# zju3dv/neuralbody

Measured on AMD Instinct MI355X. Metric: ray_samples_per_sec, higher is better.
Workload: dtype f16+f6/f4

## Files before the change

### neuralbody_amd/csrc/nb_march_common.h

```cpp
#pragma once
#include "nb_common.h"

typedef float f32x4 __attribute__((ext_vector_type(4)));
typedef float f32x16 __attribute__((ext_vector_type(16)));

namespace nbm {

constexpr int N_PE = 45;

constexpr int TAP_F = 0, TAP_H1 = 352, TAP_H2 = 608, TAP_H3 = 864, TAP_G = 1120, TAP_V = 1376, TAP_PE = 1504, TAP_WIDTH = 1600;

__device__ __forceinline__ float relu1(float x) {
    float r;
    asm("v_max_f32 %0, 0, %1" : "=v"(r) : "v"(x));
    return r;
}

__host__ __device__ constexpr int tile_row(int r, int hi) { return (r & 3) + 8 * (r >> 2) + 4 * hi; }

__host__ __device__ constexpr int lvl_c(int l) { return l == 0 ? 32 : (l == 1 ? 64 : 128); }
__host__ __device__ constexpr int lvl_chan_base(int l) { return l == 0 ? 0 : (l == 1 ? 32 : (l == 2 ? 96 : 224)); }
__host__ __device__ constexpr int lvl_reg_base(int l) { return lvl_chan_base(l) / 2; }

__host__ __device__ inline int col_feat(int q, int hi) {
// ... 106 lines not shown
    const int *ray_order;
    long long n_slots;
    float *rgb_map, *disp_map, *acc_map, *weights, *depth_map, *raw;
    long long n_rays;
    int n_samples;
    int white_bkgd;
    const float *wpts, *viewdir;
    float *raw_out, *dbg;
    long long n_pts;
    int n_wave_groups;
    float *ill;
    int ill_cap;
};

#define NB_INV_2PI 0.15915494309189533576888376337251436
__device__ __forceinline__ float sin_rev(double u) {
    const double f = u - rint(u);
    return __builtin_amdgcn_sinf((float)f);
}
__device__ __forceinline__ void pe_view(float (&pe)[N_PE], float vx, float vy, float vz, int hi) {
    const float v[3] = {vx, vy, vz};
    const double q = hi ? 0.25 : 0.0;
#pragma unroll
    for (int a = 0; a < 3; ++a) {
        const double t = (double)v[a] * NB_INV_2PI;
#pragma unroll
        for (int k = 0; k < 4; ++k) pe[3 * k + a] = sin_rev(t * (double)(1 << k) + q);
    }
}
__device__ __forceinline__ void pe_xyz(float (&pe)[N_PE], float px, float py, float pz, float vx, float vy,
                                       float vz, int hi) {
    const float p[3] = {px, py, pz};
    const float v[3] = {vx, vy, vz};
    const double q = hi ? 0.25 : 0.0;
#pragma unroll
    for (int a = 0; a < 3; ++a) {
        const double t = (double)p[a] * NB_INV_2PI;
#pragma unroll
        for (int k = 0; k < 10; ++k) pe[12 + 3 * k + a] = sin_rev(t * (double)(1 << k) + q);
    }
#pragma unroll
    for (int a = 0; a < 3; ++a) pe[42 + a] = hi ? p[a] : v[a];
}

__device__ __forceinline__ void dump_pe(const float (&pe)[N_PE], float *dst, int hi) {
#pragma unroll
    for (int c = 0; c < N_PE; ++c) dst[col_pe(c, hi) - 256] = pe[c];
}

struct GridCoord {
    float gw, gh, gd;
};

__device__ __forceinline__ GridCoord grid_coords(const SceneDev &sc, float px, float py, float pz) {
    const Pose ps = load_pose(sc.pose);
    const float qx = px - ps.Th[0], qy = py - ps.Th[1], qz = pz - ps.Th[2];
    const float cx = fmaf(qz, ps.R[6], fmaf(qy, ps.R[3], qx * ps.R[0]));
    const float cy = fmaf(qz, ps.R[7], fmaf(qy, ps.R[4], qx * ps.R[1]));
    const float cz = fmaf(qz, ps.R[8], fmaf(qy, ps.R[5], qx * ps.R[2]));
    GridCoord g;
    g.gd = __fsub_rn(__fmul_rn(__fdiv_rn(__fdiv_rn(cz - ps.bmin[2], sc.vs[0]), sc.osh[0]), 2.f), 1.f);
    g.gh = __fsub_rn(__fmul_rn(__fdiv_rn(__fdiv_rn(cy - ps.bmin[1], sc.vs[1]), sc.osh[1]), 2.f), 1.f);
    g.gw = __fsub_rn(__fmul_rn(__fdiv_rn(__fdiv_rn(cx - ps.bmin[0], sc.vs[2]), sc.osh[2]), 2.f), 1.f);
    return g;
}

template <int L>
__device__ __forceinline__ void gather_level(const SceneDev &sc, const GridCoord &g, int hi,
                                             float (&out)[lvl_c(L) / 2]) {
    constexpr int C = lvl_c(L), HALF = C / 2;
    const int D = sc.dhw[L][0], H = sc.dhw[L][1], W = sc.dhw[L][2];
    float ix = __fmul_rn(__fdiv_rn(__fadd_rn(g.gw, 1.f), 2.f), (float)(W - 1));
    float iy = __fmul_rn(__fdiv_rn(__fadd_rn(g.gh, 1.f), 2.f), (float)(H - 1));
    float iz = __fmul_rn(__fdiv_rn(__fadd_rn(g.gd, 1.f), 2.f), (float)(D - 1));
    ix = fminf(fmaxf(ix, -2.f), (float)W + 1.f);
    iy = fminf(fmaxf(iy, -2.f), (float)H + 1.f);
    iz = fminf(fmaxf(iz, -2.f), (float)D + 1.f);
    const float fx = floorf(ix), fy = floorf(iy), fz = floorf(iz);
    const int x0 = (int)fx, y0 = (int)fy, z0 = (int)fz;
    const float wx[2] = {(fx + 1.f) - ix, ix - fx};
    const float wy[2] = {(fy + 1.f) - iy, iy - fy};
    const float wz[2] = {(fz + 1.f) - iz, iz - fz};
    const float *vb = sc.vol[L] + hi * HALF;
    const f32x4 *cp[8];
    float cw[8];
#pragma unroll
    for (int corner = 0; corner < 8; ++corner) {
        const int dx = corner & 1, dy = (corner >> 1) & 1, dz = corner >> 2;
        const int xx = x0 + dx, yy = y0 + dy, zz = z0 + dz;
        const bool inb = (unsigned)xx < (unsigned)W && (unsigned)yy < (unsigned)H && (unsigned)zz < (unsigned)D;
        cw[corner] = inb ? (wx[dx] * wy[dy]) * wz[dz] : 0.f;
        const int xc = min(max(xx, 0), W - 1), yc = min(max(yy, 0), H - 1), zc = min(max(zz, 0), D - 1);
        cp[corner] = reinterpret_cast<const f32x4 *>(vb + ((size_t)(zc * H + yc) * W + xc) * C);
    }
#pragma unroll
    for (int grp = 0; grp < HALF / 16; ++grp) {
        f32x4 v[8][4];
#pragma unroll
        for (int corner = 0; corner < 8; ++corner)
#pragma unroll
            for (int q = 0; q < 4; ++q) v[corner][q] = cp[corner][grp * 4 + q];
#pragma unroll
        for (int q = 0; q < 4; ++q) {
            f32x4 a = {0.f, 0.f, 0.f, 0.f};
#pragma unroll
            for (int corner = 0; corner < 8; ++corner) {
                a.x = fmaf(cw[corner], v[corner][q].x, a.x);
                a.y = fmaf(cw[corner], v[corner][q].y, a.y);
                a.z = fmaf(cw[corner], v[corner][q].z, a.z);
                a.w = fmaf(cw[corner], v[corner][q].w, a.w);
            }
            out[grp * 16 + q * 4 + 0] = a.x;
            out[grp * 16 + q * 4 + 1] = a.y;
            out[grp * 16 + q * 4 + 2] = a.z;
            out[grp * 16 + q * 4 + 3] = a.w;
        }
// ... 318 lines not shown
```

### neuralbody_amd/csrc/nb_march_fold.hip

```cpp
#include "nb_f6_ops.h"
#include "nb_march_hooks.h"

using namespace nbm;

namespace {

#ifndef NB_FP4_TERMS
#define NB_FP4_TERMS 3
#endif
constexpr bool FP4_K[2] = {(NB_FP4_TERMS & 1) != 0, (NB_FP4_TERMS & 2) != 0};
constexpr bool ANY_FP4 = FP4_K[0] || FP4_K[1];
constexpr int TERM_ORDER[2] = {(FP4_K[0] && !FP4_K[1]) ? 1 : 0, (FP4_K[0] && !FP4_K[1]) ? 0 : 1};
__host__ __device__ constexpr int term_pieces(int k) { return FP4_K[k] ? 1 : 2; }
__host__ __device__ constexpr int block_pieces(int mt) { return (4 * mt + mt * term_pieces(0) + mt * term_pieces(1) + 1) & ~1; }
__host__ __device__ constexpr int cross_piece(int mt, int slot, int m) {
    return 4 * mt + (slot == 0 ? 0 : mt * term_pieces(TERM_ORDER[0])) + m * term_pieces(TERM_ORDER[slot]);
}
constexpr int S_R = 8;
__host__ __device__ constexpr int phase_pieces(int nb, int mt) { return nb * block_pieces(mt); }
constexpr int N_PH = 4;
constexpr int PH_NB[N_PH] = {4, 4, 4, 2};
constexpr int PH_MT[N_PH] = {2, 2, 1, 1};
__host__ __device__ constexpr int phase_p0(int ph) {
    int p = 0;
    for (int i = 0; i < ph; ++i) p += phase_pieces(PH_NB[i], PH_MT[i]);
    return p;
}
__host__ __device__ constexpr int phase_s0(int ph) {
    int n = 0;
    for (int i = 0; i < ph; ++i) n += PH_NB[i];
    return n;
}
constexpr int P_L1 = phase_p0(0), P_L2 = phase_p0(1), P_VG = phase_p0(2), P_VP = phase_p0(3), P_TOTAL = phase_p0(4);
constexpr int N_SCALE = phase_s0(4);
constexpr int WAVE_STREAM = P_TOTAL * 1024 + ((N_SCALE * 256 + 1023) & ~1023);
static_assert(P_TOTAL == (NB_FP4_TERMS == 3 ? 132 : (NB_FP4_TERMS == 0 ? 176 : 160)), "pieces per wave per depth step");
static_assert(S_R % 2 == 0 && P_L1 % 2 == 0 && P_L2 % 2 == 0 && P_VG % 2 == 0 && P_VP % 2 == 0, "six-bit fragments on even pieces");
__host__ __device__ constexpr int phase_of_p0(int p0) { return p0 == P_L1 ? 0 : (p0 == P_L2 ? 1 : (p0 == P_VG ? 2 : 3)); }

constexpr int F_OFF_B0 = 8 * 44 * 256;
constexpr int F_OFF_B1 = F_OFF_B0 + 256 + 8 * 32 * 256;
constexpr int F_OFF_B2 = F_OFF_B1 + 256 + 8 * 32 * 256;
constexpr int F_OFF_AW = F_OFF_B2 + 256;
constexpr int F_OFF_AB = F_OFF_AW + 256;
constexpr int F_OFF_L4 = F_OFF_AB + 4;
constexpr int F_OFF_LV = F_OFF_L4 + 8 * 32 * 256;
constexpr int F_OFF_BV = F_OFF_LV + 4 * 44 * 256;
constexpr int F_OFF_RW = F_OFF_BV + 128;
constexpr int F_OFF_RB = F_OFF_RW + 384;

constexpr int CH_BYTES = 2048;
constexpr int ACT16_BYTES = 16 * CH_BYTES;
constexpr int F6_BYTES = 2048;
constexpr int ACT6_OFF = ACT16_BYTES;
constexpr int ACT6_BYTES = 4 * 2 * 2 * F6_BYTES;
constexpr int ACT_BYTES = ACT6_OFF + ACT6_BYTES;
constexpr int WT_CHUNK = 4096;
constexpr int U_CHUNK = 4096;
constexpr int K_CAP = 128;
constexpr int KM_CAP = 1024;
constexpr int SCR_A = ACT_BYTES;
constexpr int SCR_C = SCR_A + 1024;
// ... 256 lines not shown

typedef short s4v __attribute__((ext_vector_type(4)));
typedef __attribute__((address_space(3))) s4v *lds_s4p;

__device__ __forceinline__ float unnorm_s(float gcoord, float fm1, float fp1) {
    const float i = __fmul_rn(__fdiv_rn(__fadd_rn(gcoord, 1.f), 2.f), fm1);
    return fminf(fmaxf(i, -2.f), fp1);
}
__device__ __forceinline__ int mad24(int a, int b, int c) {
    int r;
    asm("v_mad_i32_i24 %0, %1, %2, %3" : "=v"(r) : "v"(a), "v"(b), "v"(c));
    return r;
}
template <int N>
__device__ __forceinline__ int row_ror(int v) {
    return __builtin_amdgcn_update_dpp(v, v, 0x120 | N, 0xf, 0xf, false);
}
__device__ __forceinline__ int red_min16i(int v) {
    v = min(v, row_ror<8>(v));
    v = min(v, row_ror<4>(v));
    v = min(v, row_ror<2>(v));
    v = min(v, row_ror<1>(v));
    return v;
}
__device__ __forceinline__ int red_max16i(int v) {
    v = max(v, row_ror<8>(v));
    v = max(v, row_ror<4>(v));
    v = max(v, row_ror<2>(v));
    v = max(v, row_ror<1>(v));
    return v;
}

struct Lvl {
    int D, H, W;
    float fmx, fmy, fmz, fpx, fpy, fpz;
    const int *grid;
    int rbase;
};
__device__ __forceinline__ Lvl load_lvl(const char *actz, int part) {
    const i32x4 *p = reinterpret_cast<const i32x4 *>(actz + LC_OFF + part * 48);
    const i32x4 a = p[0], b = p[1], c = p[2];
    Lvl l;
    l.D = a.x; l.H = a.y; l.W = a.z;
    l.fmx = __int_as_float(a.w); l.fmy = __int_as_float(b.x); l.fmz = __int_as_float(b.y);
    l.fpx = __int_as_float(b.z); l.fpy = __int_as_float(b.w); l.fpz = __int_as_float(c.x);
    l.grid = reinterpret_cast<const int *>(((unsigned long long)(unsigned)c.z << 32) | (unsigned long long)(unsigned)c.y);
    l.rbase = c.w;
    return l;
}
struct LvlIdx {
    float ix, iy, iz;
    int x0, y0, z0;
};
__device__ __forceinline__ LvlIdx level_index(const Lvl &lv, const GridCoord &g) {
    LvlIdx q;
    q.ix = unnorm_s(g.gw, lv.fmx, lv.fpx);
    q.iy = unnorm_s(g.gh, lv.fmy, lv.fpy);
    q.iz = unnorm_s(g.gd, lv.fmz, lv.fpz);
    q.x0 = (int)floorf(q.ix);
    q.y0 = (int)floorf(q.iy);
    q.z0 = (int)floorf(q.iz);
    return q;
}

constexpr int BOX_BIG = 1 << 24;
__device__ __forceinline__ void prep_boxes(char *actz, const Lvl &lv, const GridCoord &g, bool take, int wslot, bool write, int os, int part) {
    const LvlIdx q = level_index(lv, g);
    int xlo = take ? min(max(q.x0, 0), lv.W - 1) : BOX_BIG, xhi = take ? min(max(q.x0 + 1, 0), lv.W - 1) : -1;
    int ylo = take ? min(max(q.y0, 0), lv.H - 1) : BOX_BIG, yhi = take ? min(max(q.y0 + 1, 0), lv.H - 1) : -1;
    int zlo = take ? min(max(q.z0, 0), lv.D - 1) : BOX_BIG, zhi = take ? min(max(q.z0 + 1, 0), lv.D - 1) : -1;
    xlo = red_min16i(xlo); ylo = red_min16i(ylo); zlo = red_min16i(zlo);
    xhi = red_max16i(xhi); yhi = red_max16i(yhi); zhi = red_max16i(zhi);
    const int any = __builtin_amdgcn_ballot_w64(take) != 0ull;
    if (write && os == 0) {
        i32x4 *d = reinterpret_cast<i32x4 *>(actz + WBOX_OFF + (wslot * 4 + part) * 32);
        d[0] = i32x4{xlo, ylo, zlo, xhi};
        d[1] = i32x4{yhi, zhi, any, 0};
    }
}

struct Prep {
    int xlo, ylo, zlo, nx, nxy, n, k0;
    int K;
    int tier;
    int any;
};
__device__ __forceinline__ int box_count(int xlo, int ylo, int zlo, int xhi, int yhi, int zhi) {
    return (xhi < xlo || yhi < ylo || zhi < zlo) ? 0 : (xhi - xlo + 1) * (yhi - ylo + 1) * (zhi - zlo + 1);
}
template <int NW>
__device__ __forceinline__ Prep prep_wg(const char *actz, int part) {
    int xlo = BOX_BIG, ylo = BOX_BIG, zlo = BOX_BIG, xhi = -1, yhi = -1, zhi = -1;
    int n16[NW], any = 0;
#pragma unroll
    for (int w = 0; w < NW; ++w) {
        const i32x4 *s = reinterpret_cast<const i32x4 *>(actz + WBOX_OFF + (w * 4 + part) * 32);
        const i32x4 a = s[0], b = s[1];
        any |= b.z;
        n16[w] = box_count(a.x, a.y, a.z, a.w, b.x, b.y);
        xlo = min(xlo, a.x); ylo = min(ylo, a.y); zlo = min(zlo, a.z);
        xhi = max(xhi, a.w); yhi = max(yhi, b.x); zhi = max(zhi, b.y);
    }
    Prep p;
    p.xlo = xlo; p.ylo = ylo; p.zlo = zlo;
    p.nx = xhi - xlo + 1;
    p.nxy = p.nx * (yhi - ylo + 1);
    p.n = box_count(xlo, ylo, zlo, xhi, yhi, zhi);
    const int n0 = __builtin_amdgcn_readlane(p.n, 0), n1 = __builtin_amdgcn_readlane(p.n, 16), n2 = __builtin_amdgcn_readlane(p.n, 32),
              n3 = __builtin_amdgcn_readlane(p.n, 48);
    p.K = n0 + n1 + n2 + n3;
    p.k0 = part == 0 ? 0 : (part == 1 ? n0 : (part == 2 ? n0 + n1 : n0 + n1 + n2));
    p.tier = 0;
    p.any = any;
    if constexpr (NW > 1) {
        if (p.K > K_CAP && p.K <= KM_CAP) {
            p.tier = 3;
        } else if (p.K > K_CAP) {
            int worst = 0;
#pragma unroll
            for (int w = 0; w < NW; ++w)
                worst = max(worst, __builtin_amdgcn_readlane(n16[w], 0) + __builtin_amdgcn_readlane(n16[w], 16) +
                                       __builtin_amdgcn_readlane(n16[w], 32) + __builtin_amdgcn_readlane(n16[w], 48));
            p.tier = worst <= K_CAP ? 1 : 2;
        }
    }
    return p;
}

struct TblLoad {
    int rid[2], idx[2];
};
__device__ __forceinline__ TblLoad tbl_issue(const Prep &p, const Lvl &lv, int wave, int os) {
    TblLoad t;
    const float rcp_xy = __builtin_amdgcn_rcpf((float)max(p.nxy, 1)), rcp_x = __builtin_amdgcn_rcpf((float)max(p.nx, 1));
#pragma unroll
    for (int q = 0; q < 2; ++q) {
        const int j = 64 * q + 16 * wave + os;
        t.rid[q] = -1;
        t.idx[q] = -1;
        if (j < p.n) {
            const int vz = (int)(((float)j + 0.5f) * rcp_xy);
            const int r = mad24(vz, -p.nxy, j);
            const int vy = (int)(((float)r + 0.5f) * rcp_x);
            const int vx = mad24(vy, -p.nx, r);
            const int lin = mad24(mad24(p.zlo + vz, lv.H, p.ylo + vy), lv.W, p.xlo + vx);
            t.rid[q] = lv.grid[lin];
            t.idx[q] = p.k0 + j;
        }
    }
    return t;
}
__device__ __forceinline__ void tbl_store(char *actz, const TblLoad &t, const Lvl &lv, unsigned zero_off, int K, int tid) {
    unsigned *tbl = reinterpret_cast<unsigned *>(actz + TBL_OFF);
#pragma unroll
    for (int q = 0; q < 2; ++q)
        if (t.idx[q] >= 0) tbl[t.idx[q]] = t.rid[q] < 0 ? zero_off : (unsigned)(lv.rbase + t.rid[q]) << 10;
    if (tid < 16 && K + tid < ((K + 15) & ~15)) tbl[K + tid] = zero_off;
}
__device__ __forceinline__ void tbl_pass(char *actz, unsigned zero_off, int k_lo, int K, int tid) {
    if (tid >= K_CAP) return;
    unsigned *tbl = reinterpret_cast<unsigned *>(actz + TBL_OFF);
    const int k = k_lo + tid;
    unsigned e = zero_off;
    if (k < K) {
        const int k1 = *reinterpret_cast<const int *>(actz + LVL_OFF + 1 * 32 + 20), k2 = *reinterpret_cast<const int *>(actz + LVL_OFF + 2 * 32 + 20),
                  k3 = *reinterpret_cast<const int *>(actz + LVL_OFF + 3 * 32 + 20);
        const int L = (k >= k1) + (k >= k2) + (k >= k3);
        const i32x4 *lp = reinterpret_cast<const i32x4 *>(actz + LVL_OFF + L * 32);
        const i32x4 b0 = lp[0], b1 = lp[1];
        const Lvl lv = load_lvl(actz, L);
        const int j = k - b1.y;
        const float rcp_xy = __builtin_amdgcn_rcpf((float)max(b1.x, 1)), rcp_x = __builtin_amdgcn_rcpf((float)max(b0.w, 1));
        const int vz = (int)(((float)j + 0.5f) * rcp_xy);
        const int r = mad24(vz, -b1.x, j);
        const int vy = (int)(((float)r + 0.5f) * rcp_x);
        const int vx = mad24(vy, -b0.w, r);
        const int lin = mad24(mad24(b0.z + vz, lv.H, b0.y + vy), lv.W, b0.x + vx);
        const int rid = lv.grid[lin];
        if (rid >= 0) e = (unsigned)(lv.rbase + rid) << 10;
    }
    tbl[tid] = e;
}
__device__ __forceinline__ void lvl_store(char *actz, const Prep &p, int tid, int os, int part) {
    if (tid < 64 && os == 0) {
        i32x4 *d = reinterpret_cast<i32x4 *>(actz + LVL_OFF + part * 32);
        d[0] = i32x4{p.xlo, p.ylo, p.zlo, p.nx};
        d[1] = i32x4{p.nxy, p.k0, p.n, 0};
    }
    if (tid == 0) *reinterpret_cast<int *>(actz + HDR_OFF) = p.K;
}

struct UCfg {
    int nch, R;
    unsigned ring;
    int ring_off;
};
__device__ __forceinline__ UCfg ucfg_k(int K, unsigned lds_base, int wave);
__device__ __forceinline__ UCfg ucfg(const char *actz, unsigned lds_base, int wave) {
    return ucfg_k(__builtin_amdgcn_readfirstlane(*reinterpret_cast<const int *>(actz + HDR_OFF)), lds_base, wave);
}
__device__ __forceinline__ UCfg ucfg_k(int K, unsigned lds_base, int wave) {
    UCfg u;
// ... 185 lines not shown
        *reinterpret_cast<f32x4 *>(irec + 4) = f32x4{z_step, __fmul_rn(1e10f, recf[11]), sigma_raw, 0.f};
    } else {
        const int ch = part - 1;
        irec[8 + ch] = part == 1 ? c0.y : (part == 2 ? c0.z : c0.w);
        irec[12 + ch] = head_sum(actz, SCR_C + (ch * 64 + sample) * 16, pk[P_RB + ch]);
    }
}

__device__ __forceinline__ void composite_step(char *actz, const float *pk, int sample, int part, float z_step, float z_after, bool last,
                                               const MarchArgs &a, long long ray, int sidx, int S, bool valid, WeightStore4 &wstore, bool ins) {
    float *recf = reinterpret_cast<float *>(actz + RAY_OFF) + sample * RAY_FLOATS;
    const f32x4 c0 = *reinterpret_cast<const f32x4 *>(recf + 12);
    const float sigma_raw = ins ? head_sum(actz, SCR_A + sample * 16, pk[P_AB]) : 0.f;
    const float d = last ? 1e10f : __fsub_rn(z_after, z_step);
    const float dist = __fmul_rn(d, recf[11]);
    const float sig = fmaxf(sigma_raw, 0.f);
    const float alpha = 1.f - expf(-sig * dist);
    const float w = alpha * c0.x;
    if (part == 0) {
        const float depth = recf[16], accw = recf[17];
        recf[12] = c0.x * (__fadd_rn(__fsub_rn(1.f, alpha), 1e-10f));
        recf[16] = fmaf(w, z_step, depth);
        recf[17] = accw + w;
    } else {
        const int ch = part - 1;
        const float o = ins ? head_sum(actz, SCR_C + (ch * 64 + sample) * 16, pk[P_RB + ch]) : 0.f;
        const float col = part == 1 ? c0.y : (part == 2 ? c0.z : c0.w);
        recf[12 + part] = fmaf(w, 1.f / (1.f + expf(-o)), col);
    }
    wstore.push(a, ray, sidx, S, part, valid, w);
    if (NB_HOOK_RAW_IS_OUTPUT && a.raw && valid && part == 0) {
        float o3[3];
#pragma unroll
        for (int ch = 0; ch < 3; ++ch) o3[ch] = ins ? head_sum(actz, SCR_C + (ch * 64 + sample) * 16, pk[P_RB + ch]) : 0.f;
        *reinterpret_cast<f32x4 *>(a.raw + (ray * S + sidx) * 4) = f32x4{o3[0], o3[1], o3[2], sigma_raw};
    }
}

__host__ __device__ inline int pe_slot_col(int a, int slot) {
    if (a >= 3 || slot >= 30) return -1;
    if (slot == 0) return 256 + 27 + a;
    if (slot <= 20) {
        const int k = (slot - 1) >> 1, is_cos = (slot - 1) & 1;
        return 256 + 27 + 3 + 6 * k + 3 * is_cos + a;
    }
    if (slot == 21) return 256 + a;
    const int k = (slot - 22) >> 1, is_cos = (slot - 22) & 1;
    return 256 + 3 + 6 * k + 3 * is_cos + a;
}

template <int MODE, bool CULL>
__global__ __launch_bounds__(256, 2) void nb_march_fold_kernel(MarchArgs a, const char *stream) {
    constexpr bool POINTS = MODE != 0, DENSITY_ONLY = MODE == 2;
    static_assert(!(CULL && POINTS), "sample culling is a property of the ray march");
    saturate_fp16_conversions();
    __shared__ __attribute__((aligned(16))) char lds[LDS_BYTES];
    char *act = lds;
    const int tid = threadIdx.x;
    const int lane = threadIdx.x & 63, wave = __builtin_amdgcn_readfirstlane(threadIdx.x >> 6);
    const int grp = xcd_remap(blockIdx.x, a.n_wave_groups);
    long long ray = (long long)grp * 64 + 16 * wave + (lane & 15);
    const long long n_units = POINTS ? a.n_pts : a.n_rays;
    bool valid = ray < n_units;
    if (!valid) ray = n_units - 1;
    if (!POINTS && a.ray_order) {
        if (a.ray_order[(long long)grp * 64] == NB_SLOT_DEAD) return;
        const int v = a.ray_order[(long long)grp * 64 + 16 * wave + (lane & 15)];
        valid = v >= 0;
        ray = valid ? v : -(long long)v - 1;
    }
    const int S = POINTS ? 1 : a.n_samples;
    {
        float ox, oy, oz, dx, dy, dz, near, far, dn, vx, vy, vz;
        if constexpr (POINTS) {
            ox = a.wpts[ray * 3 + 0], oy = a.wpts[ray * 3 + 1], oz = a.wpts[ray * 3 + 2];
            dx = DENSITY_ONLY ? 0.f : a.viewdir[ray * 3 + 0], dy = DENSITY_ONLY ? 0.f : a.viewdir[ray * 3 + 1];
            dz = DENSITY_ONLY ? 1.f : a.viewdir[ray * 3 + 2];
            near = far = 0.f;
            dn = 1.f;
            vx = dx, vy = dy, vz = dz;
        } else {
            ox = a.ray_o[ray * 3 + 0], oy = a.ray_o[ray * 3 + 1], oz = a.ray_o[ray * 3 + 2];
            dx = a.ray_d[ray * 3 + 0], dy = a.ray_d[ray * 3 + 1], dz = a.ray_d[ray * 3 + 2];
            near = a.near[ray], far = a.far[ray];
            dn = sqrtf(__fadd_rn(__fadd_rn(__fmul_rn(dx, dx), __fmul_rn(dy, dy)), __fmul_rn(dz, dz)));
            vx = dx / dn, vy = dy / dn, vz = dz / dn;
        }
        if ((lane >> 4) == 0) {
            f32x4 *rec = reinterpret_cast<f32x4 *>(lds + RAY_OFF) + (16 * wave + (lane & 15)) * (RAY_FLOATS / 4);
            rec[0] = f32x4{ox, oy, oz, near};
            rec[1] = f32x4{dx, dy, dz, far};
            rec[2] = f32x4{vx, vy, vz, dn};
            rec[3] = f32x4{1.f, 0.f, 0.f, 0.f};
            rec[4] = f32x4{0.f, 0.f, 0.f, 0.f};
        }
    }
    const float *tr = (!POINTS && a.t_rand) ? a.t_rand + ray * S : nullptr;
    auto tval = [&](int s) -> float { return ((cfloat_ptr)a.t_vals)[s]; };
    auto z_at = [&](int s, float near, float far) -> float {
        if constexpr (POINTS) return 0.f;
        const float zc = z_lin(near, far, tval(s));
        if (!tr) return zc;
        const float lower = s == 0 ? zc : 0.5f * __fadd_rn(zc, z_lin(near, far, tval(s - 1)));
        const float upper = s == S - 1 ? zc : 0.5f * __fadd_rn(z_lin(near, far, tval(s + 1)), zc);
        return __fadd_rn(lower, __fmul_rn(__fsub_rn(upper, lower), tr[s]));
    };

    {
        float *prm = reinterpret_cast<float *>(lds + PRM_OFF);
        for (int i = tid; i < P_SIZE; i += 256) {
            float v;
            if (i < P_B1) v = a.pk[F_OFF_B0 + i - P_B0];
            else if (i < P_B2) v = a.pk[F_OFF_B1 + i - P_B1];
            else if (i < P_AW) v = a.pk[F_OFF_B2 + i - P_B2];
            else if (i < P_RW) v = a.pk[F_OFF_AW + i - P_AW];
            else if (i < P_AB) v = a.pk[F_OFF_RW + i - P_RW];
            else if (i < P_RB) v = a.pk[F_OFF_AB + i - P_AB];
            else if (i < P_LB) v = a.pk[F_OFF_RB + i - P_RB];
            else v = DENSITY_ONLY ? 0.f : a.lb[256 + i - P_LB];
            prm[i] = v;
        }
        if (tid < 4) {
            int *lc = reinterpret_cast<int *>(lds + LC_OFF + tid * 48);
            const unsigned long long gp = (unsigned long long)a.fold.grid[tid];
            lc[0] = a.sc.dhw[tid][0]; lc[1] = a.sc.dhw[tid][1]; lc[2] = a.sc.dhw[tid][2];
            lc[3] = __float_as_int(a.sc.fm1[tid][2]); lc[4] = __float_as_int(a.sc.fm1[tid][1]); lc[5] = __float_as_int(a.sc.fm1[tid][0]);
            lc[6] = __float_as_int(a.sc.fp1[tid][2]); lc[7] = __float_as_int(a.sc.fp1[tid][1]); lc[8] = __float_as_int(a.sc.fp1[tid][0]);
            lc[9] = (int)(unsigned)(gp & 0xffffffffull); lc[10] = (int)(unsigned)(gp >> 32);
            lc[11] = a.fold.row_base[tid];
        }
        __syncthreads();
    }
    const __amdgpu_buffer_rsrc_t wrsrc =
        __builtin_amdgcn_make_buffer_rsrc(const_cast<char *>(stream) + (size_t)wave * WAVE_STREAM, 0, WAVE_STREAM, 0x00020000);
    WRing ring;
    WeightStore4 wstore;
    typedef void __attribute__((address_space(3))) *lptr_t;
    const unsigned lds_base = (unsigned)(unsigned long long)(lptr_t)(lds);

    float z_cur;
    GridCoord g;
    bool ins = true;
    int tier, active;
    auto prep_sequential = [&](int sn, float &z_out, int lane_c) {
        const int os = lane_c & 15, part = lane_c >> 4, sample = 16 * wave + os;
        const f32x4 *rec = reinterpret_cast<const f32x4 *>(lds + RAY_OFF) + sample * (RAY_FLOATS / 4);
        const f32x4 ro = rec[0], rd = rec[1];
        z_out = z_at(sn, ro.w, rd.w);
        const float px = __fadd_rn(ro.x, __fmul_rn(rd.x, z_out)), py = __fadd_rn(ro.y, __fmul_rn(rd.y, z_out)),
                    pz = __fadd_rn(ro.z, __fmul_rn(rd.z, z_out));
        g = grid_coords(a.sc, px, py, pz);
        if constexpr (CULL) ins = cull_inside(a.cull, a.sc, px, py, pz);
        const Lvl lv = load_lvl(lds, part);
        prep_boxes(lds, lv, g, ins, wave, true, os, part);
        __syncthreads();
        const Prep pr = prep_wg<4>(lds, part);
        tier = __builtin_amdgcn_readfirstlane(pr.tier);
        active = __builtin_amdgcn_readfirstlane(pr.any);
        if (tier == 0) {
// ... 63 lines not shown
                    lvl_store(actz, pr, tid, os, part);
                    __syncthreads();
                    const UCfg u = ucfg(actz, lds_base, wave);
                    dma_initial(a, actz, lane_i, wave, u);
                    wt_build(actz, lv, g, take, wave, os, part, u.nch);
                    __syncthreads();
                    fold_mfma(a, actz, lane_i, wave, u, acc);
                    __syncthreads();
                }
            }
            FOLD_DUMP(0, 2)
            FOLD_STAMP(2);
            ring_prime<P_L1>(wl, ring);
            publish_s(actz, lane_i, wave, acc);
            FOLD_STAMP(3);
            init_bias<2>(pk + P_B1, 2 * wave, hi, acc);
            Conv6 pec;
            {
                const f32x4 ro = rec[0], rd = rec[1], rv = rec[2];
                const float xa = part == 0 ? __fadd_rn(ro.x, __fmul_rn(rd.x, z_cur))
                                           : (part == 1 ? __fadd_rn(ro.y, __fmul_rn(rd.y, z_cur)) : __fadd_rn(ro.z, __fmul_rn(rd.z, z_cur)));
                const float va = part == 0 ? rv.x : (part == 1 ? rv.y : rv.z);
                Rev2 tx, tv;
                float e[32];
                auto pe_fill = [&](auto tc) {
                    constexpr int t = decltype(tc)::value;
                    if constexpr (t == 0) {
                        tx = rev2(xa);
                        tv = rev2(va);
                        e[0] = xa;
                        e[21] = va;
                        e[30] = 0.f;
                        e[31] = 0.f;
                    } else if constexpr (t <= 10) {
                        sincos_rev2<t - 1>(tx, e[2 * t - 1], e[2 * t]);
                    } else if constexpr (t <= 14) {
                        sincos_rev2<t - 11>(tv, e[2 * t], e[2 * t + 1]);
                    } else if constexpr (t >= 16) {
                        constexpr int i = t - 16;
                        conv6_pair<2 * i>(pec, e[4 * i], e[4 * i + 1]);
                        conv6_pair<2 * i + 1>(pec, e[4 * i + 2], e[4 * i + 3]);
                    }
                };
                if constexpr (DENSITY_ONLY) layer_s<P_L1, 2, 4, true>(wl, actz, lane_i, ring, acc);
                else layer_s<P_L1, 2, 4, true>(wl, actz, lane_i, ring, acc, pe_fill);
            }
            HalfBlock peh;
            if constexpr (!DENSITY_ONLY) peh = conv6_finish(pec);
            FOLD_DUMP(1, 2)
            FOLD_STAMP(4);
            publish_s(actz, lane_i, wave, acc);
            FOLD_STAMP(5);
            init_bias<2>(pk + P_B2, 2 * wave, hi, acc);
            layer_s<P_L2, 2, 4, true>(wl, actz, lane_i, ring, acc);
            FOLD_DUMP(2, 2)
            FOLD_STAMP(6);
            if (more) {
                const f32x4 ro = rec[0], rd = rec[1];
                z_next = z_at(s + 1, ro.w, rd.w);
                const float px = __fadd_rn(ro.x, __fmul_rn(rd.x, z_next)), py = __fadd_rn(ro.y, __fmul_rn(rd.y, z_next)),
                            pz = __fadd_rn(ro.z, __fmul_rn(rd.z, z_next));
                g = grid_coords(a.sc, px, py, pz);
                if constexpr (CULL) ins = cull_inside(a.cull, a.sc, px, py, pz);
                const Lvl lv = load_lvl(actz, part);
                prep_boxes(actz, lv, g, ins, wave, true, os, part);
            }
            FOLD_STAMP(7);
            if constexpr (DENSITY_ONLY) {
#pragma unroll
                for (int m = 0; m < 2; ++m)
#pragma unroll
                    for (int n = 0; n < 2; ++n)
#pragma unroll
                        for (int r = 0; r < 16; ++r) acc[m][n][r] = relu1(acc[m][n][r]);
            } else {
                publish_s(actz, lane_i, wave, acc);
            }
            FOLD_STAMP(8);
            {
#pragma unroll
                for (int n = 0; n < 2; ++n) {
                    float s4[4] = {0.f, 0.f, 0.f, 0.f};
#pragma unroll
                    for (int m = 0; m < 2; ++m) {
                        const f32x4 *aw = reinterpret_cast<const f32x4 *>(pk + P_AW + hi * 128 + 16 * (2 * wave + m));
#pragma unroll
                        for (int q4 = 0; q4 < 4; ++q4) {
                            const f32x4 w4 = aw[q4];
                            s4[0] = fmaf(w4.x, acc[m][n][4 * q4 + 0], s4[0]);
                            s4[1] = fmaf(w4.y, acc[m][n][4 * q4 + 1], s4[1]);
                            s4[2] = fmaf(w4.z, acc[m][n][4 * q4 + 2], s4[2]);
                            s4[3] = fmaf(w4.w, acc[m][n][4 * q4 + 3], s4[3]);
                        }
                    }
                    float sa = add_halves((s4[0] + s4[1]) + (s4[2] + s4[3]));
                    if (hi == 0) reinterpret_cast<float *>(actz + SCR_A)[(n * 32 + (lane_i & 31)) * 4 + wave] = sa;
                }
            }
            if constexpr (!DENSITY_ONLY) {
                TblLoad tl;
                int k_next = 0;
                if (more) {
                    const Lvl lv = load_lvl(actz, part);
                    const Prep pr = prep_wg<4>(actz, part);
                    tier_next = __builtin_amdgcn_readfirstlane(pr.tier);
                    active_next = __builtin_amdgcn_readfirstlane(pr.any);
                    k_next = __builtin_amdgcn_readfirstlane(pr.K);
                    tl.rid[0] = tl.rid[1] = tl.idx[0] = tl.idx[1] = -1;
                    if (tier_next == 0) tl = tbl_issue(pr, lv, wave, os);
                    lvl_store(actz, pr, tid, os, part);
                }
                FOLD_STAMP(9);
                init_bias<1>(pk + P_LB, wave, hi, acc);
                layer_s<P_VG, 1, 4, false>(wl, actz, lane_i, ring, acc);
                FOLD_STAMP(10);
                if (more && tier_next == 0) {
                    const Lvl lv = load_lvl(actz, part);
                    tbl_store(actz, tl, lv, a.fold.zero_off, k_next, tid);
                }
                __syncthreads();
                ring_prime<P_VP>(wl, ring);
                store_halfblock(actz, part >> 1, part & 1, sn, ss, peh);
                __syncthreads();
                FOLD_STAMP(11);
                layer_s<P_VP, 1, 2, false>(wl, actz, lane_i, ring, acc);
                FOLD_STAMP(12);
                FOLD_DUMP(3, 1)
                {
#pragma unroll
                    for (int n = 0; n < 2; ++n) {
                        float rl[16];
#pragma unroll
                        for (int r = 0; r < 16; ++r) rl[r] = relu1(acc[0][n][r]);
#pragma unroll
                        for (int ch = 0; ch < 3; ++ch) {
                            const f32x4 *rw = reinterpret_cast<const f32x4 *>(pk + P_RW + (ch * 2 + hi) * 64 + 16 * wave);
                            float c4[4] = {0.f, 0.f, 0.f, 0.f};
#pragma unroll
                            for (int q4 = 0; q4 < 4; ++q4) {
                                const f32x4 w4 = rw[q4];
                                c4[0] = fmaf(w4.x, rl[4 * q4 + 0], c4[0]);
                                c4[1] = fmaf(w4.y, rl[4 * q4 + 1], c4[1]);
                                c4[2] = fmaf(w4.z, rl[4 * q4 + 2], c4[2]);
                                c4[3] = fmaf(w4.w, rl[4 * q4 + 3], c4[3]);
                            }
                            float sc = add_halves((c4[0] + c4[1]) + (c4[2] + c4[3]));
                            if (hi == 0) reinterpret_cast<float *>(actz + SCR_C)[(ch * 64 + n * 32 + (lane_i & 31)) * 4 + wave] = sc;
                        }
                    }
                }
            }
        } else if (more) {
            prep_sequential(s + 1, z_next, lane_i);
            tier_next = tier;
            active_next = active;
        }
        FOLD_STAMP(13);
        __syncthreads();
        FOLD_STAMP(14);
        if (more) {
            tier = tier_next;
            active = active_next;
            fetch_and_weights(lane_i);
        }
        FOLD_STAMP(15);
        {
            if constexpr (POINTS) {
// ... 289 lines not shown
```

Measured before the change: 1.399 billion.

## Interleave next-sample coordinate and box prep into MFMA layer loops

Splits the next-sample position, grid-coordinate and per-axis box computation into small steps and passes them as fill callbacks into the FC2 layer loop. It also splits the workgroup box merge, k-list prep and table gather issue into steps run inside the VG layer loop. The aim is to hide scalar and latency-bound work under matrix instructions instead of running it serially between layers. The cost is higher register pressure and a more complex schedule, and the change depends on layer_s accepting a fill functor, which is not shown.

```diff
diff --git a/neuralbody_amd/csrc/nb_march_common.h b/neuralbody_amd/csrc/nb_march_common.h
--- a/neuralbody_amd/csrc/nb_march_common.h
+++ b/neuralbody_amd/csrc/nb_march_common.h
@@ -182,16 +182,26 @@
     float gw, gh, gd;
 };
 
-__device__ __forceinline__ GridCoord grid_coords(const SceneDev &sc, float px, float py, float pz) {
+struct CanonRel {
+    float d, h, w;
+};
+__device__ __forceinline__ CanonRel grid_canon_rel(const SceneDev &sc, float px, float py, float pz) {
     const Pose ps = load_pose(sc.pose);
     const float qx = px - ps.Th[0], qy = py - ps.Th[1], qz = pz - ps.Th[2];
     const float cx = fmaf(qz, ps.R[6], fmaf(qy, ps.R[3], qx * ps.R[0]));
     const float cy = fmaf(qz, ps.R[7], fmaf(qy, ps.R[4], qx * ps.R[1]));
     const float cz = fmaf(qz, ps.R[8], fmaf(qy, ps.R[5], qx * ps.R[2]));
+    return CanonRel{cz - ps.bmin[2], cy - ps.bmin[1], cx - ps.bmin[0]};
+}
+__device__ __forceinline__ float grid_axis_voxels(float rel, float vs) { return __fdiv_rn(rel, vs); }
+__device__ __forceinline__ float grid_axis_norm(float voxels, float osh) { return __fsub_rn(__fmul_rn(__fdiv_rn(voxels, osh), 2.f), 1.f); }
+
+__device__ __forceinline__ GridCoord grid_coords(const SceneDev &sc, float px, float py, float pz) {
+    const CanonRel c = grid_canon_rel(sc, px, py, pz);
     GridCoord g;
-    g.gd = __fsub_rn(__fmul_rn(__fdiv_rn(__fdiv_rn(cz - ps.bmin[2], sc.vs[0]), sc.osh[0]), 2.f), 1.f);
-    g.gh = __fsub_rn(__fmul_rn(__fdiv_rn(__fdiv_rn(cy - ps.bmin[1], sc.vs[1]), sc.osh[1]), 2.f), 1.f);
-    g.gw = __fsub_rn(__fmul_rn(__fdiv_rn(__fdiv_rn(cx - ps.bmin[0], sc.vs[2]), sc.osh[2]), 2.f), 1.f);
+    g.gd = grid_axis_norm(grid_axis_voxels(c.d, sc.vs[0]), sc.osh[0]);
+    g.gh = grid_axis_norm(grid_axis_voxels(c.h, sc.vs[1]), sc.osh[1]);
+    g.gw = grid_axis_norm(grid_axis_voxels(c.w, sc.vs[2]), sc.osh[2]);
     return g;
 }
 
diff --git a/neuralbody_amd/csrc/nb_march_fold.hip b/neuralbody_amd/csrc/nb_march_fold.hip
--- a/neuralbody_amd/csrc/nb_march_fold.hip
+++ b/neuralbody_amd/csrc/nb_march_fold.hip
@@ -8,6 +8,10 @@
 #ifndef NB_FP4_TERMS
 #define NB_FP4_TERMS 3
 #endif
+#ifndef NB_MARCH_FILLS
+#define NB_MARCH_FILLS 3
+#endif
+constexpr bool FILL_FC2 = (NB_MARCH_FILLS & 1) != 0, FILL_VG = (NB_MARCH_FILLS & 2) != 0;
 constexpr bool FP4_K[2] = {(NB_FP4_TERMS & 1) != 0, (NB_FP4_TERMS & 2) != 0};
 constexpr bool ANY_FP4 = FP4_K[0] || FP4_K[1];
 constexpr int TERM_ORDER[2] = {(FP4_K[0] && !FP4_K[1]) ? 1 : 0, (FP4_K[0] && !FP4_K[1]) ? 0 : 1};
@@ -370,31 +374,63 @@
     float ix, iy, iz;
     int x0, y0, z0;
 };
+__device__ __forceinline__ void level_axis(float gcoord, float fm1, float fp1, float &i, int &i0) {
+    i = unnorm_s(gcoord, fm1, fp1);
+    i0 = (int)floorf(i);
+}
 __device__ __forceinline__ LvlIdx level_index(const Lvl &lv, const GridCoord &g) {
     LvlIdx q;
-    q.ix = unnorm_s(g.gw, lv.fmx, lv.fpx);
-    q.iy = unnorm_s(g.gh, lv.fmy, lv.fpy);
-    q.iz = unnorm_s(g.gd, lv.fmz, lv.fpz);
-    q.x0 = (int)floorf(q.ix);
-    q.y0 = (int)floorf(q.iy);
-    q.z0 = (int)floorf(q.iz);
+    level_axis(g.gw, lv.fmx, lv.fpx, q.ix, q.x0);
+    level_axis(g.gh, lv.fmy, lv.fpy, q.iy, q.y0);
+    level_axis(g.gd, lv.fmz, lv.fpz, q.iz, q.z0);
     return q;
 }
 
 constexpr int BOX_BIG = 1 << 24;
+struct Box {
+    int xlo, ylo, zlo, xhi, yhi, zhi;
+};
+__device__ __forceinline__ void box_clamp(int i0, int size, bool take, int &lo, int &hi) {
+    lo = take ? min(max(i0, 0), size - 1) : BOX_BIG;
+    hi = take ? min(max(i0 + 1, 0), size - 1) : -1;
+}
+__device__ __forceinline__ int wave_takes_any(bool take) { return __builtin_amdgcn_ballot_w64(take) != 0ull; }
 __device__ __forceinline__ void prep_boxes(char *actz, const Lvl &lv, const GridCoord &g, bool take, int wslot, bool write, int os, int part) {
     const LvlIdx q = level_index(lv, g);
-    int xlo = take ? min(max(q.x0, 0), lv.W - 1) : BOX_BIG, xhi = take ? min(max(q.x0 + 1, 0), lv.W - 1) : -1;
-    int ylo = take ? min(max(q.y0, 0), lv.H - 1) : BOX_BIG, yhi = take ? min(max(q.y0 + 1, 0), lv.H - 1) : -1;
-    int zlo = take ? min(max(q.z0, 0), lv.D - 1) : BOX_BIG, zhi = take ? min(max(q.z0 + 1, 0), lv.D - 1) : -1;
-    xlo = red_min16i(xlo); ylo = red_min16i(ylo); zlo = red_min16i(zlo);
-    xhi = red_max16i(xhi); yhi = red_max16i(yhi); zhi = red_max16i(zhi);
-    const int any = __builtin_amdgcn_ballot_w64(take) != 0ull;
+    Box b;
+    box_clamp(q.x0, lv.W, take, b.xlo, b.xhi);
+    box_clamp(q.y0, lv.H, take, b.ylo, b.yhi);
+    box_clamp(q.z0, lv.D, take, b.zlo, b.zhi);
+    b.xlo = red_min16i(b.xlo); b.ylo = red_min16i(b.ylo); b.zlo = red_min16i(b.zlo);
+    b.xhi = red_max16i(b.xhi); b.yhi = red_max16i(b.yhi); b.zhi = red_max16i(b.zhi);
+    const int any = wave_takes_any(take);
     if (write && os == 0) {
         i32x4 *d = reinterpret_cast<i32x4 *>(actz + WBOX_OFF + (wslot * 4 + part) * 32);
-        d[0] = i32x4{xlo, ylo, zlo, xhi};
-        d[1] = i32x4{yhi, zhi, any, 0};
-    }
+        d[0] = i32x4{b.xlo, b.ylo, b.zlo, b.xhi};
+        d[1] = i32x4{b.yhi, b.zhi, any, 0};
+    }
+}
+template <int AX>
+__device__ __forceinline__ void box_axis_own(const char *actz, int part, float gcoord, bool take, int &lo, int &hi) {
+    const int *lc = reinterpret_cast<const int *>(actz + LC_OFF + part * 48);
+    float i;
+    int i0;
+    level_axis(gcoord, __int_as_float(lc[3 + AX]), __int_as_float(lc[6 + AX]), i, i0);
+    box_clamp(i0, lc[2 - AX], take, lo, hi);
+}
+template <int AX>
+__device__ __forceinline__ void box_axis_store(char *actz, int lo, int hi, int wslot, bool write, int os, int part) {
+    lo = red_min16i(lo);
+    hi = red_max16i(hi);
+    if (write && os == 0) {
+        int *d = reinterpret_cast<int *>(actz + WBOX_OFF + (wslot * 4 + part) * 32);
+        d[AX] = lo;
+        d[3 + AX] = hi;
+    }
+}
+__device__ __forceinline__ void box_any_store(char *actz, bool take, int wslot, bool write, int os, int part) {
+    const int any = wave_takes_any(take);
+    if (write && os == 0) reinterpret_cast<int *>(actz + WBOX_OFF + (wslot * 4 + part) * 32)[6] = any;
 }
 
 struct Prep {
@@ -407,18 +443,32 @@
     return (xhi < xlo || yhi < ylo || zhi < zlo) ? 0 : (xhi - xlo + 1) * (yhi - ylo + 1) * (zhi - zlo + 1);
 }
 template <int NW>
+struct WgBox {
+    Box b = {BOX_BIG, BOX_BIG, BOX_BIG, -1, -1, -1};
+    int n16[NW], any = 0;
+};
+template <int NW>
+__device__ __forceinline__ void wg_box_merge(const char *actz, int part, int w, WgBox<NW> &m) {
+    const i32x4 *s = reinterpret_cast<const i32x4 *>(actz + WBOX_OFF + (w * 4 + part) * 32);
+    const i32x4 a = s[0], b = s[1];
+    m.any |= b.z;
+    m.n16[w] = box_count(a.x, a.y, a.z, a.w, b.x, b.y);
+    m.b.xlo = min(m.b.xlo, a.x); m.b.ylo = min(m.b.ylo, a.y); m.b.zlo = min(m.b.zlo, a.z);
+    m.b.xhi = max(m.b.xhi, a.w); m.b.yhi = max(m.b.yhi, b.x); m.b.zhi = max(m.b.zhi, b.y);
+}
+template <int NW>
+__device__ __forceinline__ Prep prep_wg_finish(const WgBox<NW> &m, int part);
+template <int NW>
 __device__ __forceinline__ Prep prep_wg(const char *actz, int part) {
-    int xlo = BOX_BIG, ylo = BOX_BIG, zlo = BOX_BIG, xhi = -1, yhi = -1, zhi = -1;
-    int n16[NW], any = 0;
-#pragma unroll
-    for (int w = 0; w < NW; ++w) {
-        const i32x4 *s = reinterpret_cast<const i32x4 *>(actz + WBOX_OFF + (w * 4 + part) * 32);
-        const i32x4 a = s[0], b = s[1];
-        any |= b.z;
-        n16[w] = box_count(a.x, a.y, a.z, a.w, b.x, b.y);
-        xlo = min(xlo, a.x); ylo = min(ylo, a.y); zlo = min(zlo, a.z);
-        xhi = max(xhi, a.w); yhi = max(yhi, b.x); zhi = max(zhi, b.y);
-    }
+    WgBox<NW> m;
+#pragma unroll
+    for (int w = 0; w < NW; ++w) wg_box_merge(actz, part, w, m);
+    return prep_wg_finish(m, part);
+}
+template <int NW>
+__device__ __forceinline__ Prep prep_wg_finish(const WgBox<NW> &m, int part) {
+    const int xlo = m.b.xlo, ylo = m.b.ylo, zlo = m.b.zlo, xhi = m.b.xhi, yhi = m.b.yhi, zhi = m.b.zhi, any = m.any;
+    const int(&n16)[NW] = m.n16;
     Prep p;
     p.xlo = xlo; p.ylo = ylo; p.zlo = zlo;
     p.nx = xhi - xlo + 1;
@@ -448,24 +498,25 @@
 struct TblLoad {
     int rid[2], idx[2];
 };
+__device__ __forceinline__ void tbl_issue_one(TblLoad &t, int q, const Prep &p, const Lvl &lv, int wave, int os) {
+    const float rcp_xy = __builtin_amdgcn_rcpf((float)max(p.nxy, 1)), rcp_x = __builtin_amdgcn_rcpf((float)max(p.nx, 1));
+    const int j = 64 * q + 16 * wave + os;
+    t.rid[q] = -1;
+    t.idx[q] = -1;
+    if (j < p.n) {
+        const int vz = (int)(((float)j + 0.5f) * rcp_xy);
+        const int r = mad24(vz, -p.nxy, j);
+        const int vy = (int)(((float)r + 0.5f) * rcp_x);
+        const int vx = mad24(vy, -p.nx, r);
+        const int lin = mad24(mad24(p.zlo + vz, lv.H, p.ylo + vy), lv.W, p.xlo + vx);
+        t.rid[q] = lv.grid[lin];
+        t.idx[q] = p.k0 + j;
+    }
+}
 __device__ __forceinline__ TblLoad tbl_issue(const Prep &p, const Lvl &lv, int wave, int os) {
     TblLoad t;
-    const float rcp_xy = __builtin_amdgcn_rcpf((float)max(p.nxy, 1)), rcp_x = __builtin_amdgcn_rcpf((float)max(p.nx, 1));
-#pragma unroll
-    for (int q = 0; q < 2; ++q) {
-        const int j = 64 * q + 16 * wave + os;
-        t.rid[q] = -1;
-        t.idx[q] = -1;
-        if (j < p.n) {
-            const int vz = (int)(((float)j + 0.5f) * rcp_xy);
-            const int r = mad24(vz, -p.nxy, j);
-            const int vy = (int)(((float)r + 0.5f) * rcp_x);
-            const int vx = mad24(vy, -p.nx, r);
-            const int lin = mad24(mad24(p.zlo + vz, lv.H, p.ylo + vy), lv.W, p.xlo + vx);
-            t.rid[q] = lv.grid[lin];
-            t.idx[q] = p.k0 + j;
-        }
-    }
+    tbl_issue_one(t, 0, p, lv, wave, os);
+    tbl_issue_one(t, 1, p, lv, wave, os);
     return t;
 }
 __device__ __forceinline__ void tbl_store(char *actz, const TblLoad &t, const Lvl &lv, unsigned zero_off, int K, int tid) {
@@ -757,6 +808,7 @@
 template <int MODE, bool CULL>
 __global__ __launch_bounds__(256, 2) void nb_march_fold_kernel(MarchArgs a, const char *stream) {
     constexpr bool POINTS = MODE != 0, DENSITY_ONLY = MODE == 2;
+    constexpr bool FILL_KLIST = FILL_VG && !CULL;
     static_assert(!(CULL && POINTS), "sample culling is a property of the ray march");
     saturate_fp16_conversions();
     __shared__ __attribute__((aligned(16))) char lds[LDS_BYTES];
@@ -802,14 +854,15 @@
     }
     const float *tr = (!POINTS && a.t_rand) ? a.t_rand + ray * S : nullptr;
     auto tval = [&](int s) -> float { return ((cfloat_ptr)a.t_vals)[s]; };
-    auto z_at = [&](int s, float near, float far) -> float {
+    auto z_at_t = [&](int s, float near, float far, float trs) -> float {
         if constexpr (POINTS) return 0.f;
         const float zc = z_lin(near, far, tval(s));
         if (!tr) return zc;
         const float lower = s == 0 ? zc : 0.5f * __fadd_rn(zc, z_lin(near, far, tval(s - 1)));
         const float upper = s == S - 1 ? zc : 0.5f * __fadd_rn(z_lin(near, far, tval(s + 1)), zc);
-        return __fadd_rn(lower, __fmul_rn(__fsub_rn(upper, lower), tr[s]));
+        return __fadd_rn(lower, __fmul_rn(__fsub_rn(upper, lower), trs));
     };
+    auto z_at = [&](int s, float near, float far) -> float { return z_at_t(s, near, far, (!POINTS && tr) ? tr[s] : 0.f); };
 
     {
         float *prm = reinterpret_cast<float *>(lds + PRM_OFF);
@@ -979,10 +1032,60 @@
             publish_s(actz, lane_i, wave, acc);
             FOLD_STAMP(5);
             init_bias<2>(pk + P_B2, 2 * wave, hi, acc);
-            layer_s<P_L2, 2, 4, true>(wl, actz, lane_i, ring, acc);
+            if constexpr (POINTS || !FILL_FC2) {
+                layer_s<P_L2, 2, 4, true>(wl, actz, lane_i, ring, acc);
+            } else {
+                const int s1 = more ? s + 1 : s;
+                f32x4 ro, rd;
+                float trn = 0.f, px, py, pz, vox;
+                CanonRel cr;
+                int lo, hi2;
+                auto next_fill = [&](auto tc) {
+                    constexpr int t = decltype(tc)::value;
+                    if constexpr (t == 0) {
+                        ro = rec[0], rd = rec[1];
+                        if (tr) trn = tr[s1];
+                    } else if constexpr (t == 1) {
+                        z_next = z_at_t(s1, ro.w, rd.w, trn);
+                        px = __fadd_rn(ro.x, __fmul_rn(rd.x, z_next)), py = __fadd_rn(ro.y, __fmul_rn(rd.y, z_next)),
+                        pz = __fadd_rn(ro.z, __fmul_rn(rd.z, z_next));
+                    } else if constexpr (t == 2) {
+                        if constexpr (CULL) ins = cull_inside(a.cull, a.sc, px, py, pz);
+                    } else if constexpr (t == 3) {
+                        cr = grid_canon_rel(a.sc, px, py, pz);
+                    } else if constexpr (t == 4) {
+                        vox = grid_axis_voxels(cr.d, a.sc.vs[0]);
+                    } else if constexpr (t == 5) {
+                        g.gd = grid_axis_norm(vox, a.sc.osh[0]);
+                    } else if constexpr (t == 6) {
+                        box_axis_own<2>(actz, part, g.gd, ins, lo, hi2);
+                    } else if constexpr (t == 7) {
+                        box_axis_store<2>(actz, lo, hi2, wave, more, os, part);
+                    } else if constexpr (t == 8) {
+                        vox = grid_axis_voxels(cr.h, a.sc.vs[1]);
+                    } else if constexpr (t == 9) {
+                        g.gh = grid_axis_norm(vox, a.sc.osh[1]);
+                    } else if constexpr (t == 10) {
+                        box_axis_own<1>(actz, part, g.gh, ins, lo, hi2);
+                    } else if constexpr (t == 11) {
+                        box_axis_store<1>(actz, lo, hi2, wave, more, os, part);
+                    } else if constexpr (t == 12) {
+                        vox = grid_axis_voxels(cr.w, a.sc.vs[2]);
+                    } else if constexpr (t == 13) {
+                        g.gw = grid_axis_norm(vox, a.sc.osh[2]);
+                    } else if constexpr (t == 14) {
+                        box_axis_own<0>(actz, part, g.gw, ins, lo, hi2);
+                    } else if constexpr (t == 15) {
+                        box_axis_store<0>(actz, lo, hi2, wave, more, os, part);
+                    } else if constexpr (t == 16) {
+                        box_any_store(actz, ins, wave, more, os, part);
+                    }
+                };
+                layer_s<P_L2, 2, 4, true>(wl, actz, lane_i, ring, acc, next_fill);
+            }
             FOLD_DUMP(2, 2)
             FOLD_STAMP(6);
-            if (more) {
+            if (!FILL_FC2 && more) {
                 const f32x4 ro = rec[0], rd = rec[1];
                 z_next = z_at(s + 1, ro.w, rd.w);
                 const float px = __fadd_rn(ro.x, __fmul_rn(rd.x, z_next)), py = __fadd_rn(ro.y, __fmul_rn(rd.y, z_next)),
@@ -1026,20 +1129,44 @@
             }
             if constexpr (!DENSITY_ONLY) {
                 TblLoad tl;
+                tl.rid[0] = tl.rid[1] = tl.idx[0] = tl.idx[1] = -1;
                 int k_next = 0;
-                if (more) {
+                if (!FILL_KLIST && more) {
                     const Lvl lv = load_lvl(actz, part);
                     const Prep pr = prep_wg<4>(actz, part);
                     tier_next = __builtin_amdgcn_readfirstlane(pr.tier);
                     active_next = __builtin_amdgcn_readfirstlane(pr.any);
                     k_next = __builtin_amdgcn_readfirstlane(pr.K);
-                    tl.rid[0] = tl.rid[1] = tl.idx[0] = tl.idx[1] = -1;
                     if (tier_next == 0) tl = tbl_issue(pr, lv, wave, os);
                     lvl_store(actz, pr, tid, os, part);
                 }
                 FOLD_STAMP(9);
                 init_bias<1>(pk + P_LB, wave, hi, acc);
-                layer_s<P_VG, 1, 4, false>(wl, actz, lane_i, ring, acc);
+                if constexpr (POINTS || !FILL_KLIST) {
+                    layer_s<P_VG, 1, 4, false>(wl, actz, lane_i, ring, acc);
+                } else {
+                    Lvl lv;
+                    WgBox<4> wb;
+                    Prep pr;
+                    auto klist_fill = [&](auto tc) {
+                        constexpr int t = decltype(tc)::value;
+                        if constexpr (t < 4) {
+                            wg_box_merge(actz, part, t, wb);
+                        } else if constexpr (t == 4) {
+                            pr = prep_wg_finish(wb, part);
+                        } else if constexpr (t == 5) {
+                            tier_next = __builtin_amdgcn_readfirstlane(pr.tier);
+                            active_next = __builtin_amdgcn_readfirstlane(pr.any);
+                            k_next = __builtin_amdgcn_readfirstlane(pr.K);
+                            if (more) lvl_store(actz, pr, tid, os, part);
+                        } else if constexpr (t == 6) {
+                            lv = load_lvl(actz, part);
+                        } else if constexpr (t == 7 || t == 8) {
+                            if (more && tier_next == 0) tbl_issue_one(tl, t - 7, pr, lv, wave, os);
+                        }
+                    };
+                    layer_s<P_VG, 1, 4, false>(wl, actz, lane_i, ring, acc, klist_fill);
+                }
                 FOLD_STAMP(10);
                 if (more && tier_next == 0) {
                     const Lvl lv = load_lvl(actz, part);
```

Measured after the change: 1.403 billion, median of 6. No clear change (+0.3%).
